# OpenGene/fastplong

Measured on AMD Instinct MI355X. Metric: Gbases/s processed (trim+cut+filter), higher is better.
Workload: dtype u8; 1 GPU; c3_full_pipeline: BASELINE.json configs[2] -- 1000000 synthetic reads per GPU, lognormal lengths (median 8000, sigma 0.5, N50 ~10 kb), Q~N(18,8), -s/-e fixed, --cut_front --cut_tail -W 5, -x, -y; inputs resident in HBM; reads_per_gpu=1000000, bases_per_gpu=9061022094, max_read_len=99450, parallelism=shard1 (independent read shards, one RCCL all-reduce of the counters)

## Files before the change

### fastplong_amd/csrc/dev_prims.h

```cpp
#ifndef FPL_DEV_PRIMS_H
#define FPL_DEV_PRIMS_H

#include <stdint.h>

#ifdef FPL_EMU
#include "hip_emu.h"
#else
#include <hip/hip_runtime.h>
#endif

#ifdef FPL_EMU
#define FPL_NOINLINE
#else
#define FPL_NOINLINE __attribute__((noinline))
#endif

namespace fpl {

constexpr int WAVE = 64;

typedef unsigned long long u64;
typedef uint32_t u32;
typedef uint8_t u8;

// ... 199 lines not shown
    u32 r = 0;
    for (int i = 0; i < 32; i++) {
        const int idx = (((a >> i) & 1) << 2) | (((b >> i) & 1) << 1) | ((c >> i) & 1);
        r |= (u32)((TT >> idx) & 1) << i;
    }
    return r;
#else
    return __builtin_amdgcn_bitop3_b32(a, b, c, TT);
#endif
}
__device__ __forceinline__ void csa(u32& h, u32& l, u32 a, u32 b, u32 c) {
    const u32 hh = bitop3<0xE8>(a, b, c);
    l = bitop3<0x96>(a, b, c);
    h = hh;
}

__device__ __forceinline__ u32 udot4(u32 a, u32 b, u32 c) {
#ifdef FPL_EMU
    u32 r = c;
    for (int i = 0; i < 4; i++) r += ((a >> (8 * i)) & 0xFF) * ((b >> (8 * i)) & 0xFF);
    return r;
#else
    return __builtin_amdgcn_udot4(a, b, c, false);
#endif
}
__device__ __forceinline__ void dot_settle(u32& a, u32& b) {
#ifndef FPL_EMU
    asm volatile("s_nop 3" : "+v"(a), "+v"(b));
#else
    (void)a;
    (void)b;
#endif
}
__device__ __forceinline__ u32 sum_bytes(u32 a, u32 c) {
#ifdef FPL_EMU
    return c + (a & 0xFF) + ((a >> 8) & 0xFF) + ((a >> 16) & 0xFF) + (a >> 24);
#else
    return __builtin_amdgcn_sad_u8(a, 0u, c);
#endif
}
__device__ __forceinline__ u32 perm_lo(u32 tbl, u32 sel) {
#ifdef FPL_EMU
    u32 r = 0;
    for (int i = 0; i < 4; i++) {
        const u32 k = (sel >> (8 * i)) & 0xFF;
        r |= ((k < 4 ? (tbl >> (8 * k)) : 0) & 0xFF) << (8 * i);
    }
    return r;
#else
    return __builtin_amdgcn_perm(0u, tbl, sel);
#endif
}
__device__ __forceinline__ u32 perm_b32(u32 hi, u32 lo, u32 sel) {
#ifdef FPL_EMU
    const u64 v = ((u64)hi << 32) | lo;
    u32 r = 0;
    for (int i = 0; i < 4; i++) {
        const u32 k = (sel >> (8 * i)) & 0xFF;
        r |= (u32)((k < 8 ? (v >> (8 * k)) : 0) & 0xFF) << (8 * i);
    }
    return r;
#else
    return __builtin_amdgcn_perm(hi, lo, sel);
#endif
}
__device__ __forceinline__ u32 uniform_u32(u32 v) {
// ... 76 lines not shown
```

### fastplong_amd/csrc/dev_types.h

```cpp
#ifndef FPL_DEV_TYPES_H
#define FPL_DEV_TYPES_H

#include <math.h>
#include <stdint.h>
#include <string.h>

#include "../../include/fastplong_amd.h"

namespace fpl {

constexpr int PEQ_WORDS = 4;

struct DevAdapter {
    int32_t len;
    int32_t plen;
    uint8_t seq[256];
    uint32_t seqw[256];
    uint32_t peq16_start[256];
    uint32_t peq16_end[256];
    uint64_t peq_full[256][PEQ_WORDS];
    uint32_t term[64];
    int32_t acgt_only;
    uint32_t onehot[8];
    uint64_t peq4_full[4];
    uint32_t peq4_s16[4];
    uint32_t peq4_e16[4];
    uint32_t peq4_e32[4];
    uint32_t peq4_s32r[4];
};

struct DevConfig {
    int32_t trim_front, trim_tail;
    int32_t cut_front, cut_tail;
    int32_t cut_front_w, cut_front_thr;
    int32_t cut_tail_w, cut_tail_thr;
    int32_t polyx, polyx_min_len;
    int32_t adapter_enabled, ext;
    int32_t has_start, has_end, n_fasta;
    int32_t trim_mode;
    int32_t qual_filter, qualified_qual, unqual_pct, n_base_limit, n_pct_limit, avg_qual_req;
    int32_t length_filter, required_length, max_length;
    int32_t complexity, complexity_pct;
    int32_t brk, brk_w, brk_thr, msk, msk_w, msk_thr, defer;
    int32_t dbg;
    int32_t ham_fast;
    int32_t scan_short;
    int32_t thr[FPL_MAX_ADAPTER_LEN + 1];
};

struct ReadState {
    uint32_t s, e;
    uint32_t dropped;
    uint32_t pad;
};

inline void build_adapter(DevAdapter* a, const char* seq, int len) {
    memset(a, 0, sizeof(*a));
    a->len = len;
    a->plen = len < FPL_PATTERN_LEN ? len : FPL_PATTERN_LEN;
    for (int i = 0; i < len; i++) {
        uint8_t c = (uint8_t)seq[i];
        a->seq[i] = c;
        a->seqw[i] = 0x01010101u * c;
        a->peq_full[c][i >> 6] |= 1ull << (i & 63);
    }
    a->acgt_only = len <= 64;
    for (int i = 0; i < 64; i++) a->term[i] = (4u * 4u * 64u) << 8;
    for (int i = 0; i < len && i < 64; i++) {
        const uint8_t c = (uint8_t)seq[i];
        if (c != 'A' && c != 'C' && c != 'G' && c != 'T') a->acgt_only = 0;
        const uint32_t code = (c >> 1) & 3u;
        a->term[i] = ((4u * (code * 64u + (uint32_t)(i >> 5))) << 8) | (uint32_t)(i & 31);
    }
    for (int i = 0; i < len && i < 64; i++) {
        const uint8_t c = (uint8_t)seq[i];
        const uint32_t nib = c == 'A' ? 1u : (c == 'C' ? 2u : (c == 'G' ? 4u : (c == 'T' ? 8u : 0u)));
        a->onehot[i >> 3] |= nib << (4 * (i & 7));
    }
    for (int j = 0; j < a->plen; j++) {
        a->peq16_start[(uint8_t)seq[len - a->plen + j]] |= 1u << j;
        a->peq16_end[(uint8_t)seq[j]] |= 1u << j;
    }
    {
        static const uint8_t letters[4] = {'A', 'C', 'T', 'G'};
        for (int c = 0; c < 4; c++) {
            a->peq4_full[c] = a->peq_full[letters[c]][0];
            a->peq4_s16[c] = a->peq16_start[letters[c]];
            a->peq4_e16[c] = a->peq16_end[letters[c]];
            a->peq4_e32[c] = 0;
            a->peq4_s32r[c] = 0;
            const int m = len < 32 ? len : 32;
            for (int i = 0; i < m; i++) {
                if ((uint8_t)seq[i] == letters[c]) a->peq4_e32[c] |= 1u << i;
                if ((uint8_t)seq[len - 1 - i] == letters[c]) a->peq4_s32r[c] |= 1u << i;
            }
        }
    }
}

inline int trim_mode_of(const int* lens, const int* acgt_only, int n_adapters) {
    bool short_ok = n_adapters == 2, mid_ok = true;
    for (int i = 0; i < n_adapters; i++) {
        const int l = lens[i];
        if (l == 0 && i < 2) continue;
        if (l < 16 || l > 32 || !acgt_only[i]) short_ok = false;
// ... 47 lines not shown
```

### fastplong_amd/csrc/kernels.h

```cpp
#ifndef FPL_KERNELS_H
#define FPL_KERNELS_H

#include "adapter_pick.h"
#include "dev_prims.h"
#include "dev_types.h"

namespace fpl {

#if defined(FPL_PROF) && !defined(FPL_EMU)
__device__ unsigned long long g_fpl_prof[64];
#define PROF_INIT()                                     \
    unsigned long long prof_a[12] = {0, 0, 0, 0, 0, 0, 0, 0, 0, 0, 0, 0}; \
    unsigned long long prof_t = __builtin_amdgcn_s_memtime()
#define PROF(i)                                                     \
    {                                                               \
        const unsigned long long t_ = __builtin_amdgcn_s_memtime(); \
        prof_a[i] += t_ - prof_t;                                   \
        prof_t = t_;                                                \
    }
#define PROF_FLUSH(base)                                                                      \
    if (lane_id() == 0)                                                                       \
        for (int i_ = 0; i_ < 12; i_++) atomicAdd(&g_fpl_prof[(base) + i_], prof_a[i_])
#else
#define PROF_INIT()
// ... 1468 lines not shown
        cC += (c == 'C' || c == 'N');
        cG += (c == 'G' || c == 'N');
        const int cmp = pos + 1, allowed = min(5, cmp / 8);
        const bool need = (cmp - cA > allowed) && (cmp - cT > allowed) && (cmp - cC > allowed) && (cmp - cG > allowed);
        if (need && (pos >= 8 || pos + 1 >= compareReq - 1)) {
            P = pos;
            break;
        }
        pos++;
        if (++it > LANE_SCAN_CAP) slow = true;
    }
    if (!active || slow || P + 1 < compareReq) return rlen;
    int poly = 0, maxc = cA;
    if (cT > maxc) { maxc = cT; poly = 1; }
    if (cC > maxc) { maxc = cC; poly = 2; }
    if (cG > maxc) { maxc = cG; poly = 3; }
    const u32 polyBase = poly == 0 ? 'A' : (poly == 1 ? 'T' : (poly == 2 ? 'C' : 'G'));
    int i = rlen - P - 1;
    if (i < 0) i = 0;
    it = 0;
    while (i < rlen && r[i] != polyBase) {
        i++;
        if (++it > LANE_SCAN_CAP) {
            slow = true;
            return rlen;
        }
    }
    const int p2 = i < rlen ? rlen - i - 1 : -1;
    poly_out = poly;
    trimmed_out = p2 + 1;
    return rlen - p2 - 1;
}

__device__ __forceinline__ u32 onehot4(u32 w) {
    const u32 code = (w >> 1) & 0x03030303u;
    const u32 t = perm_lo(0x47544341u, code) ^ w;
    const u32 ok = (~(((t & 0x7F7F7F7Fu) + 0x7F7F7F7Fu) | t) >> 7) & 0x01010101u;
    const u32 nib = perm_lo(0x04080201u, code) & (ok * 15u);
    const u32 h = (nib | (nib >> 4)) & 0x00FF00FFu;
    return (h | (h >> 8)) & 0xFFFFu;
}
template <bool START, int NW = 4>
__device__ __forceinline__ void ham_scan_lanes(const u8* __restrict__ r1, int rlen, bool active, const u32 (&ad1h)[NW], int alen,
                                               int thr, const u8* __restrict__ seq_end, int& hit, int& cand) {
    hit = -1;
    cand = -1;
    int p_lo = 0, np = 0;
    if (START) {
        const int searchEnd = min(rlen, FPL_END_WINDOW);
        if (active && alen <= rlen && searchEnd > alen) np = searchEnd - alen + 1;
    } else {
        const int ss = max(0, rlen - FPL_END_WINDOW);
        if (active && ss + alen <= rlen) {
            p_lo = ss;
            np = rlen - alen - ss;
        }
    }
    const int npmax = (int)wave_max_u32((u32)max(np, 0));
    if (npmax == 0) return;
    const u8* base = r1 + p_lo;
    const int navail = np > 0 ? rlen - p_lo : 0;
    auto nibbles = [&](int k) -> u32 {
        const int left = navail - 4 * k;
        if (left <= 0) return 0u;
        u32 w = load4_guard(base + 4 * k, seq_end);
        if (left < 4) w &= (1u << (8 * left)) - 1u;
        return onehot4(w);
    };
    u32 touch = 0;
    if (navail > 64)
        touch = (u32)*(base + min(navail - 1, 112)) + (u32)*(base + min(navail - 1, 207));
    u32 W[NW];
#pragma unroll
    for (int k = 0; k < NW; k++) W[k] = nibbles(2 * k) | (nibbles(2 * k + 1) << 16);
    int bestmm = 0x7fffffff;
    u32 nxt = nibbles(2 * NW);
    for (int i0 = 0; i0 < npmax; i0 += 4) {
        const u32 cur = nxt;
        nxt = nibbles(i0 / 4 + 2 * NW + 1);
#pragma unroll
        for (int u = 0; u < 4; u++) {
            const int i = i0 + u;
            u32 matches = popc32(W[0] & ad1h[0]);
#pragma unroll
            for (int k = 1; k < NW; k++) matches = popc_acc(W[k] & ad1h[k], matches);
            const int mm = alen - (int)matches;
            const bool in = i < np;
            const int p = p_lo + i;
            if (START) {
                hit = (in && mm <= thr) ? p : hit;
                const bool better = in && mm < bestmm;
                cand = better ? p : cand;
                bestmm = better ? mm : bestmm;
            } else {
                hit = (in && hit < 0 && mm <= thr) ? p : hit;
                const bool better = in && mm <= bestmm;
                cand = better ? p : cand;
                bestmm = better ? mm : bestmm;
            }
#pragma unroll
            for (int k = 0; k + 1 < NW; k++) W[k] = alignbit(W[k + 1], W[k], 4);
            W[NW - 1] = (W[NW - 1] >> 4) | (((cur >> (4 * u)) & 15u) << 28);
        }
    }
    if (hit >= 0) cand = -1;
#if !defined(FPL_EMU)
    asm volatile("" ::"v"(touch));
#else
    (void)touch;
#endif
}

__device__ __forceinline__ bool lev_lanes32(const u8* __restrict__ text, int m, int shift, int thr, bool need,
                                            const uint64_t (*__restrict__ peqf)[1], const u8* __restrict__ seq_end) {
    u32 w[8] = {0, 0, 0, 0, 0, 0, 0, 0};
    if (need) {
        const u32x4 a = load16_guard(text, seq_end), b = load16_guard(text + 16, seq_end);
        w[0] = a.x; w[1] = a.y; w[2] = a.z; w[3] = a.w;
        w[4] = b.x; w[5] = b.y; w[6] = b.z; w[7] = b.w;
    }
    const int mm = need ? m : 0;
    const u32 mask = mm >= 32 ? ~0u : ((1u << mm) - 1u);
    const u32 topsh = mm > 0 ? (u32)(mm - 1) : 0u;
    const int mmax = (int)wave_max_u32((u32)mm);
    u32 Pv = ~0u, Mv = 0;
    int score = mm;
#pragma unroll
    for (int t = 0; t < 32; t++) {
        if (t < mmax) {
            const u32 c = (w[t >> 2] >> (8 * (t & 3))) & 0xFFu;
            const u32 Eq = (u32)(peqf[c][0] >> shift) & mask;
            const u32 Xv = Eq | Mv;
            const u32 Xh = (((Eq & Pv) + Pv) ^ Pv) | Eq;
            u32 Ph = Mv | ~(Xh | Pv);
            u32 Mh = Pv & Xh;
            const int sc = score + (int)((Ph >> topsh) & 1u) - (int)((Mh >> topsh) & 1u);
            Ph = (Ph << 1) | 1u;
            Mh <<= 1;
            const bool act = t < mm;
            score = act ? sc : score;
            const u32 nPv = Mh | ~(Xv | Ph), nMv = Ph & Xv;
            Pv = act ? nPv : Pv;
            Mv = act ? nMv : Mv;
        }
// ... 159 lines not shown
        if (ok && ed <= thrP) {
            if (START) {
                if (ed < mined) {
                    mined = ed;
                    pos = p;
                }
            } else if (pos < 0 || ed <= mined) {
                pos = p;
                mined = ed;
            } else {
                stop = true;
            }
        }
        if (stop) {
            cur = 0;
            nz = 0;
        }
    }
    return pos;
}

__device__ __forceinline__ int lane_get(int v, int j) { return readlane_i32(v, j); }
__device__ __forceinline__ void lane_set(int& v, int j, int x) { v = lane_id() == j ? x : v; }

#ifndef FPL_TRIM_WAVES_PER_SIMD_BATCHED
#define FPL_TRIM_WAVES_PER_SIMD_BATCHED 5
#endif
template <int WAVES, int NW = 4, bool CHAIN = false>
__global__ void __launch_bounds__(WAVES * 64, FPL_TRIM_WAVES_PER_SIMD_BATCHED)
k_trim_ends_batched(const u8* __restrict__ seq, const u8* __restrict__ qual, const uint64_t* __restrict__ off, u32 n_reads,
                    uint64_t n_bytes, const DevConfig* __restrict__ cfg, const DevAdapter* __restrict__ ads,
                    ReadState* __restrict__ state, long long* __restrict__ counters, u32 C, u32* __restrict__ group_ctr) {
    __shared__ TrimBlockAcc acc;
    __shared__ TrimLds<WAVES> lds;
    __shared__ int thr_lds[72];
    __shared__ u32 cand_lds[WAVES][PART_WORDS][64];
    PROF_INIT();
    const int lane = lane_id();
    u32(*const cand)[64] = cand_lds[wave_in_block()];
    for (u32 i = threadIdx.x; i < FPL_FR_LEN; i += blockDim.x) acc.fr[i] = 0;
    for (u32 i = threadIdx.x; i < 2 * 2 * FPL_KEY_STRIDE; i += blockDim.x) acc.key[i] = 0;
    for (u32 i = threadIdx.x; i < 256; i += blockDim.x) {
        lds.peq16[0][i] = (uint16_t)ads[0].peq16_start[i];
        lds.peq16[1][i] = (uint16_t)ads[1].peq16_end[i];
        lds.peqf[0][i][0] = ads[0].peq_full[i][0];
        lds.peqf[1][i][0] = ads[1].peq_full[i][0];
    }
    for (u32 i = threadIdx.x; i < 72; i += blockDim.x) thr_lds[i] = i <= 64 ? cfg->thr[i] : 0;
    __syncthreads();
    const u8* seq_end = seq + n_bytes;
    const u8* qual_end = qual + n_bytes;
    u32* const win_s = lds.win[wave_in_block()][0];
    u32* const win_e = lds.win[wave_in_block()][1];
    u32* const win_hq = lds.win[wave_in_block()][2];
    u32* const win_tq = lds.win[wave_in_block()][3];
    u32* const win4_s = lds.win4[wave_in_block()][0];
    u32* const win4_e = lds.win4[wave_in_block()][1];
    const bool do_ad = cfg->adapter_enabled != 0;
    const bool do_start = do_ad && cfg->has_start, do_end = do_ad && cfg->has_end;
    const int ext = cfg->ext;
    const int alen0 = ads[0].len, alen1 = ads[1].len;
    constexpr int plen = FPL_PATTERN_LEN;
    const int thrA0 = cfg->thr[alen0], thrA1 = cfg->thr[alen1], thrP = cfg->thr[plen];
    u32 ad1h0[NW], ad1h1[NW];
#pragma unroll
    for (int k = 0; k < NW; k++) {
        ad1h0[k] = uniform_u32(ads[0].onehot[k]);
        ad1h1[k] = uniform_u32(ads[1].onehot[k]);
    }

    const u32 n_groups = (n_reads + 63) / 64;
    for (;;) {
        u32 grp = 0;
        if (lane == 0) grp = atomicAdd(group_ctr, 1u);
        grp = readlane_u32(grp, 0);
        if (grp >= n_groups) break;
        const u32 g0 = grp * 64;
        const int gn = (int)min(64u, n_reads - g0);
        FPL_TRIM_STAT(0, 1);
        uint64_t v_o0 = 0;
        int v_l = 0;
        if (lane < gn) {
            v_o0 = off[g0 + lane];
            v_l = (int)(off[g0 + lane + 1] - v_o0);
        }
        int v_s = 0, v_e = 0, v_alive = 0, v_trim = 0;
        int v_mpos = -1;
        int v_cand = -1;

        PROF(0)
        bool v_slow = false;
        {
            bool alive = false, slow = false;
            const bool wide = (cfg->cut_front && cfg->cut_front_w > LANE_SCAN_WMAX) || (cfg->cut_tail && cfg->cut_tail_w > LANE_SCAN_WMAX);
            if (!wide) {
                trim_and_cut_lanes(seq + v_o0, qual + v_o0, v_l, lane < gn, cfg, v_s, v_e, alive, slow);
                if (cfg->polyx) {
                    int poly, tl;
                    const int nl = trim_polyx_lanes(seq + v_o0 + v_s, v_e - v_s, alive && !slow, cfg->polyx_min_len, poly, tl, slow);
                    if (!slow) {
                        v_e = v_s + nl;
                        if (poly >= 0) {
// ... 9 lines not shown
            v_slow = slow;
        }
        PROF(1)
        for (u64 todo = wave_ballot(v_slow); todo;) {
            const int j = __ffsll(todo) - 1;
            todo &= todo - 1;
            FPL_TRIM_STAT(1, 1);
            const uint64_t o0 = readlane_u64(v_o0, j);
            const int l = lane_get(v_l, j);
            const u8* sq = seq + o0;
            const u8* ql = qual + o0;
            const int tail0 = max(0, l - TRIM_WIN);
            stage_ends<true>(win_s, win_e, win_hq, win_tq, win4_s, win4_e, sq, ql, l, tail0, seq_end, qual_end);
            const EndsView vs = {sq, (const u8*)win_s, (const u8*)win_e, tail0};
            const EndsView vq = {ql, (const u8*)win_hq, (const u8*)win_tq, tail0};
            int s, e;
            const bool alive = trim_and_cut_wave(vs, vq, l, cfg, s, e);
            if (alive && cfg->polyx) {
                int poly, tl;
                const int nl = trim_polyx_wave(vs, s, e - s, cfg->polyx_min_len, poly, tl);
                e = s + nl;
                if (poly >= 0 && lane == 0) {
                    atomicAdd(&acc.fr[FPL_FR_POLYX_READS + poly], (u64)1);
                    atomicAdd(&acc.fr[FPL_FR_POLYX_BASES + poly], (u64)tl);
                }
            }
            lane_set(v_s, j, s);
            lane_set(v_e, j, e);
            lane_set(v_alive, j, alive ? 1 : 0);
        }
        PROF(2)
        if (do_start) {
            const bool act = v_alive && (v_e - v_s) >= FPL_PATTERN_LEN;
            ham_scan_lanes<true, NW>(seq + v_o0 + v_s, v_e - v_s, act, ad1h0, alen0, thrA0, seq_end, v_mpos, v_cand);
        }
        PROF(3)
        if (do_start) {
            const bool need = v_cand >= 0;
            FPL_TRIM_STAT(2, __popcll(wave_ballot(need)));
            if (wave_ballot(need)) {
                const bool ok = lev_lanes_nw<NW>(seq + v_o0 + v_s + v_cand, alen0, 0, thrA0, need, lds.peqf[0], seq_end);
                v_mpos = ok ? v_cand : v_mpos;
            }
        }
        PROF(4)
        int v_ppos = -1;
        if (do_start) {
            const int rl = v_e - v_s;
            const bool wants = v_alive && v_mpos < 0 && rl >= FPL_PATTERN_LEN;
            bool may = false;
            if (wave_ballot(wants)) {
                const int n = min(rl, FPL_END_WINDOW);
                const u32 nzc = partial16_candidates(seq + v_o0 + v_s, n, thrP, wants, lds.peq16[0], seq_end, cand);
                if (wave_ballot(nzc != 0))
                    v_ppos = partial16_resolve_lanes<true>(seq + v_o0 + v_s, n, min(rl - plen, FPL_END_WINDOW - plen), thrP, nzc,
                                                           lds.peq16[0], seq_end, cand, may);
            }
            u64 todo = wave_ballot(may);
            FPL_TRIM_STAT(3, __popcll(wave_ballot(wants)));
            FPL_TRIM_STAT(4, __popcll(todo));
            while (todo) {
                const int j = __ffsll(todo) - 1;
                todo &= todo - 1;
                const uint64_t o0 = readlane_u64(v_o0, j);
                const int s = lane_get(v_s, j), e = lane_get(v_e, j), rlen = e - s;
                const u8* sq = seq + o0;
                stage_window(win_s, sq + s, min(rlen, FPL_END_WINDOW), seq_end, nullptr);
// ... 18 lines not shown
            }
        }
        PROF(5)
        if (do_start) {
            const int rlen = v_e - v_s;
            const int cmplen = min(v_ppos + plen, alen0);
            const bool need = v_ppos >= 0;
            bool pok = false;
            if (wave_ballot(need))
                pok = lev_lanes_nw<NW>(seq + v_o0 + v_s + v_ppos + plen - cmplen, cmplen, alen0 - cmplen, thr_lds[need ? cmplen : 0], need,
                                  lds.peqf[0], seq_end);
            int kl = 0, got = 0;
            if (v_mpos >= 0) {
                const int mp = min(v_mpos + ext, rlen - alen0);
                kl = alen0;
                v_s += min(rlen - 1, mp + alen0);
                got = mp + alen0;
            } else if (pok) {
                const int pos = min(v_ppos + ext, rlen - alen0);
                kl = cmplen;
                const int n = min(rlen - 1, pos + plen);
                if (n < 0) v_s = v_e;
                else v_s += n;
                got = pos + plen;
            }
            v_trim += got;
            if (kl > 0) atomicAdd(&acc.key[(0 * 2 + 0) * FPL_KEY_STRIDE + kl], 1u);
        }
        PROF(6)
        v_mpos = -1;
        v_cand = -1;
        if (do_end) {
            const bool act = v_alive && (v_e - v_s) >= FPL_PATTERN_LEN;
            ham_scan_lanes<false, NW>(seq + v_o0 + v_s, v_e - v_s, act, ad1h1, alen1, thrA1, seq_end, v_mpos, v_cand);
        }
        PROF(7)
        if (do_end) {
            const bool need = v_cand >= 0;
            FPL_TRIM_STAT(5, __popcll(wave_ballot(need)));
            if (wave_ballot(need)) {
                const bool ok = lev_lanes_nw<NW>(seq + v_o0 + v_s + v_cand, alen1, 0, thrA1, need, lds.peqf[1], seq_end);
                v_mpos = ok ? v_cand : v_mpos;
            }
        }
        PROF(8)
        v_ppos = -1;
        if (do_end) {
            const int rl = v_e - v_s, wlf = min(rl, FPL_END_WINDOW);
            const bool wants = v_alive && v_mpos < 0 && rl >= FPL_PATTERN_LEN;
            bool may = false;
            if (wave_ballot(wants)) {
                const u32 nzc = partial16_candidates(seq + v_o0 + v_e - wlf, wlf, thrP, wants, lds.peq16[1], seq_end, cand);
                if (wave_ballot(nzc != 0)) {
                    const int pos = partial16_resolve_lanes<false>(seq + v_o0 + v_e - 16, wlf, min(rl - plen, FPL_END_WINDOW - plen), thrP,
                                                                   nzc, lds.peq16[1], seq_end, cand, may);
                    v_ppos = pos > 0 ? pos : -1;
                }
            }
            u64 todo = wave_ballot(may);
            FPL_TRIM_STAT(6, __popcll(wave_ballot(wants)));
            FPL_TRIM_STAT(7, __popcll(todo));
            while (todo) {
                const int j = __ffsll(todo) - 1;
                todo &= todo - 1;
                const uint64_t o0 = readlane_u64(v_o0, j);
                const int s = lane_get(v_s, j), e = lane_get(v_e, j), rlen = e - s;
                const u8* sq = seq + o0;
// ... 46 lines not shown
                v_e = v_s + mp;
                got = rlen - mp;
            } else if (pok) {
                const int pos = min(v_ppos + ext, rlen - plen);
                kl = cmplen;
                v_e = v_s + (rlen - plen - pos);
                got = pos + plen;
            }
            v_trim += got;
            if (kl > 0) atomicAdd(&acc.key[(1 * 2 + 1) * FPL_KEY_STRIDE + kl], 1u);
        }
        if (do_ad && !CHAIN) {
            const u64 nt = wave_ballot(v_trim > 0);
            const u32 tb = wave_sum_u32(v_trim > 0 ? (u32)v_trim : 0u);
            if (nt && lane == 0) {
                atomicAdd(&acc.fr[FPL_FR_ADAPTER_READS], (u64)__popcll(nt));
                atomicAdd(&acc.fr[FPL_FR_ADAPTER_BASES], (u64)tb);
            }
        }
        if (lane < gn) {
            ReadState st;
            st.s = v_alive ? (u32)v_s : 0;
            st.e = v_alive ? (u32)v_e : 0;
            st.dropped = v_alive ? 0 : 1;
            st.pad = CHAIN ? (u32)v_trim : 0u;
            state[g0 + lane] = st;
        }
        PROF(10)
    }
    PROF_FLUSH(32);
    __syncthreads();
    long long* fr = counters + FPL_OFF_FR(C);
    long long* keyh = counters + FPL_OFF_KEYHIST(C);
    for (u32 i = threadIdx.x; i < FPL_FR_LEN; i += blockDim.x)
        if (acc.fr[i]) atomicAdd((u64*)&fr[i], acc.fr[i]);
    for (u32 i = threadIdx.x; i < 2 * 2 * FPL_KEY_STRIDE; i += blockDim.x)
        if (acc.key[i]) atomicAdd((u64*)&keyh[i], (u64)acc.key[i]);
}

constexpr int FS_T = 512;
constexpr int FS_SMAX = 96;
constexpr int FS_PT = FS_T + FS_SMAX;
constexpr int FS_SLAB = 8 * FS_T + 8 * FS_PT;
constexpr int FS_STRIDE = FS_T + FS_PT;
__device__ __forceinline__ u32 fs_pre_cell(u32 i) { return (i / FS_T) * FS_STRIDE + (i % FS_T); }
__device__ __forceinline__ u32 fs_post_cell(u32 j) { return (j / FS_PT) * FS_STRIDE + FS_T + (j % FS_PT); }
constexpr u32 CS_MAX_ITEMS_PER_SLICE = 16383;
#ifndef FPL_ABL
#define FPL_ABL 0
#endif
constexpr int CS_GROUP = 4;
constexpr u32 PLAN_TO_POST = 1u;

__device__ __forceinline__ u32 kmer_codes(u32 d) { return (d & 0x02020202u) | ((d >> 2) & 0x01010101u); }
__device__ __forceinline__ u32 kmer_pack(u32 v) {
    const u32 x = lshl_or<10>(v, v);
    return lshl_or<20>(x, x);
}
__device__ __forceinline__ u32 kmer_pack_dot(u32 v) { return udot4(v, 0x01041040u, 0u); }
__device__ __forceinline__ u32 kmer_stream(u32 v0, u32 v1, u32 pack_h0) {
    u32 p0 = kmer_pack_dot(v0), p1 = kmer_pack_dot(v1);
    dot_settle(p0, p1);
    const u32 W01 = lshl_or<8>(p0, p1);
    return lshl_or<16>(wave_prev_u32(W01, pack_h0), W01);
}
__device__ __forceinline__ u32 invalid_nibble(u32 mapped, u32 d) {
    const u32 x = (mapped ^ d) & ~((mapped >> 4) & 0x01010101u);
    const u32 nz = (((x & 0x7F7F7F7Fu) + 0x7F7F7F7Fu) | x) & 0x80808080u;
    const u32 y = lshl_or<7>(nz, nz);
// ... 499 lines not shown
                    const u32 mm = (acc[j >> 2] >> (8 * (j & 3))) & 0xFF;
                    if (j0 + j < npos0 && mm < bmm0) {
                        bmm0 = mm;
                        bp0 = (u32)(j0 + j);
                    }
                }
            }
            if (npos1 > t0) {
                hamming16(rb + a + j0, seq_end, sv, ad1->seqw, ad1->len, acc);
#pragma unroll
                for (int j = 0; j < 16; j++) {
                    const u32 mm = (acc[j >> 2] >> (8 * (j & 3))) & 0xFF;
                    if (j0 + j < npos1 && mm < bmm1) {
                        bmm1 = mm;
                        bp1 = (u32)(j0 + j);
                    }
                }
            }
        }
    }
    if (SUMS) {
        sums.lowq = wave_sum_u32(lowq);
        sums.nn = wave_sum_u32(nn);
        sums.totq = wave_sum_u32(totq);
        sums.diff = wave_sum_u32(diff);
    }
    if (HAM) {
        key0 = wave_min_u64(((u64)bmm0 << 32) | bp0);
        key1 = wave_min_u64(((u64)bmm1 << 32) | bp1);
    }
}


__device__ __forceinline__ void code_planes(const u32 s[8], u32& L, u32& H, u32& N) {
    L = 0;
    H = 0;
    N = 0;
#pragma unroll
    for (int pr = 0; pr < 4; pr++) {
        u32 lb = 0, hb = 0, nb = 0;
#pragma unroll
        for (int hh = 0; hh < 2; hh++) {
            const u32 w = s[2 * pr + hh];
            const u32 wt = hh ? 0x80402010u : 0x08040201u;
            lb = udot4(w & 0x02020202u, wt, lb);
            hb = udot4(w & 0x04040404u, wt, hb);
            nb = udot4(w & 0x08080808u, wt, nb);
        }
        L |= pr ? lb << (8 * pr - 1) : lb >> 1;
        H |= pr ? hb << (8 * pr - 2) : hb >> 2;
        N |= pr ? nb << (8 * pr - 3) : nb >> 3;
    }
}
__device__ __forceinline__ u32 not_acgtn(const u32 s[8]) {
    u32 bad = 0;
#pragma unroll
    for (int d = 0; d < 8; d++) bad |= perm_b32(0x4E000000u, 0x47544341u, (s[d] >> 1) & 0x07070707u) ^ s[d];
    return bad;
}
template <bool MASKED, bool QS = true>
__device__ __forceinline__ void sums32_acgtn(const u32 s0, const u32 q[8], int nvalid, u32 L, u32 H, u32 N, u32 prev_dword,
                                             u32 qqrep, u32& lowq, u32& nn, u32& totq, u32& diff) {
#pragma unroll
    for (int d = 0; QS && d < 8; d++) {
        u32 bm = ~0u, fm = 0x80808080u;
        if (MASKED) {
            const int c = nvalid - 4 * d;
            bm = c >= 4 ? ~0u : (c <= 0 ? 0u : ((1u << (8 * c)) - 1u));
            fm &= bm;
        }
        const u32 t = (q[d] | 0x80808080u) - qqrep;
        lowq = popc_acc(~t & fm, lowq);
        totq = sum_bytes(q[d] & bm, totq);
    }
    const u32 vm = (!MASKED || nvalid >= 32) ? ~0u : ((1u << nvalid) - 1u);
    nn = popc_acc(N & vm, nn);
    const u32 dm = ((L ^ (L << 1)) | (H ^ (H << 1)) | (N ^ (N << 1))) & ~1u & vm;
    const u32 d0 = ((s0 & 0xFFu) != (prev_dword >> 24)) ? 1u : 0u;
    diff = popc_acc(dm, diff) + d0;
}
__device__ __forceinline__ void build_planes(const u32 s[8], u32& PA, u32& PC, u32& PT, u32& PG) {
    u32 L = 0, H = 0, X = 0;
#pragma unroll
    for (int pr = 0; pr < 4; pr++) {
        u32 lb = 0, hb = 0, xb = 0;
#pragma unroll
        for (int hh = 0; hh < 2; hh++) {
            const u32 w = s[2 * pr + hh];
            const u32 wt = hh ? 0x80402010u : 0x08040201u;
            const u32 w1 = w >> 1;
            lb = udot4(w1 & 0x01010101u, wt, lb);
            hb = udot4((w >> 2) & 0x01010101u, wt, hb);
            const u32 e = perm_lo(0x47544341u, w1 & 0x03030303u);
            const u32 t = e ^ w;
            const u32 nz = ((((t & 0x7F7F7F7Fu) + 0x7F7F7F7Fu) | t) >> 7) & 0x01010101u;
            xb = udot4(nz, wt, xb);
        }
        L |= lb << (8 * pr);
        H |= hb << (8 * pr);
        X |= xb << (8 * pr);
    }
    const u32 V = ~X;
    PA = bitop3<0x10>(V, H, L);
    PC = bitop3<0x20>(V, H, L);
    PT = bitop3<0x40>(V, H, L);
    PG = bitop3<0x80>(V, H, L);
}

template <int NB>
__device__ __forceinline__ void match_counts(const u32* __restrict__ plane_lane, const DevAdapter* __restrict__ ad, u32 (&B)[NB]) {
    const int alen = ad->len;
#ifndef FPL_EMU
    const u32 planes_m0 = uniform_u32((u32)(size_t)plane_lane - 4u * (u32)lane_id());
#endif
#pragma unroll
    for (int b = 0; b < NB; b++) B[b] = 0;
    auto group8 = [&](int i0) -> u32 {
        u32 m[8], tw[8];
#pragma unroll
        for (int k = 0; k < 8; k++) tw[k] = ad->term[i0 + k];
#ifdef FPL_EMU
#pragma unroll
        for (int k = 0; k < 8; k++) {
            const u32* p = plane_lane + (tw[k] >> 10);
            m[k] = alignbit(p[1], p[0], tw[k] & 31u);
        }
#else
        u32 lo[8], hi[8], m0_keep;
        asm volatile(
            "s_mov_b32 %16, m0\n"
            "s_lshr_b32 m0, %17, 8\n s_add_u32 m0, m0, %25\n s_nop 0\n ds_read_addtid_b32 %0 offset:0\n ds_read_addtid_b32 %8 offset:4\n"
            "s_lshr_b32 m0, %18, 8\n s_add_u32 m0, m0, %25\n s_nop 0\n ds_read_addtid_b32 %1 offset:0\n ds_read_addtid_b32 %9 offset:4\n"
            "s_lshr_b32 m0, %19, 8\n s_add_u32 m0, m0, %25\n s_nop 0\n ds_read_addtid_b32 %2 offset:0\n ds_read_addtid_b32 %10 offset:4\n"
            "s_lshr_b32 m0, %20, 8\n s_add_u32 m0, m0, %25\n s_nop 0\n ds_read_addtid_b32 %3 offset:0\n ds_read_addtid_b32 %11 offset:4\n"
            "s_lshr_b32 m0, %21, 8\n s_add_u32 m0, m0, %25\n s_nop 0\n ds_read_addtid_b32 %4 offset:0\n ds_read_addtid_b32 %12 offset:4\n"
            "s_lshr_b32 m0, %22, 8\n s_add_u32 m0, m0, %25\n s_nop 0\n ds_read_addtid_b32 %5 offset:0\n ds_read_addtid_b32 %13 offset:4\n"
            "s_lshr_b32 m0, %23, 8\n s_add_u32 m0, m0, %25\n s_nop 0\n ds_read_addtid_b32 %6 offset:0\n ds_read_addtid_b32 %14 offset:4\n"
            "s_lshr_b32 m0, %24, 8\n s_add_u32 m0, m0, %25\n s_nop 0\n ds_read_addtid_b32 %7 offset:0\n ds_read_addtid_b32 %15 offset:4\n"
            "s_waitcnt lgkmcnt(0)\n s_mov_b32 m0, %16"
            : "=&v"(lo[0]), "=&v"(lo[1]), "=&v"(lo[2]), "=&v"(lo[3]), "=&v"(lo[4]), "=&v"(lo[5]), "=&v"(lo[6]), "=&v"(lo[7]),
              "=&v"(hi[0]), "=&v"(hi[1]), "=&v"(hi[2]), "=&v"(hi[3]), "=&v"(hi[4]), "=&v"(hi[5]), "=&v"(hi[6]), "=&v"(hi[7]),
              "=&s"(m0_keep)
            : "s"(tw[0]), "s"(tw[1]), "s"(tw[2]), "s"(tw[3]), "s"(tw[4]), "s"(tw[5]), "s"(tw[6]), "s"(tw[7]), "s"(planes_m0)
            : "scc", "memory");
        (void)m0_keep;
#pragma unroll
        for (int k = 0; k < 8; k++) m[k] = alignbit(hi[k], lo[k], tw[k]);
#endif
        u32 t1, t2, t3, t4, f1, f2, e;
        csa(t1, B[0], B[0], m[0], m[1]);
        csa(t2, B[0], B[0], m[2], m[3]);
        csa(f1, B[1], B[1], t1, t2);
        csa(t3, B[0], B[0], m[4], m[5]);
        csa(t4, B[0], B[0], m[6], m[7]);
        csa(f2, B[1], B[1], t3, t4);
        csa(e, B[2], B[2], f1, f2);
        return e;
    };
    auto ripple = [&](u32 c, int lvl) {
#pragma unroll
        for (int b = 3; b < NB; b++) {
            if (b < lvl) continue;
            const u32 t = B[b] & c;
            B[b] ^= c;
            c = t;
        }
    };
    int i0 = 0;
    for (; i0 + 8 < alen; i0 += 16) {
        const u32 ea = group8(i0);
        const u32 eb = group8(i0 + 8);
        u32 c16;
        csa(c16, B[3], B[3], ea, eb);
        ripple(c16, 4);
    }
    for (; i0 < alen; i0 += 8) ripple(group8(i0), 3);
}

template <int NB>
__device__ __forceinline__ void sliced_max(const u32 (&B)[NB], u32 cand, int& val, int& first) {
    val = 0;
#pragma unroll
    for (int b = NB - 1; b >= 0; b--) {
        const u32 t = cand & B[b];
        const bool nz = t != 0;
        cand = nz ? t : cand;
#ifndef FPL_EMU
        {
            u64 c = wave_ballot(nz);
            asm("s_nop 1\n\tv_addc_co_u32_e64 %0, %1, %0, %0, %1" : "+v"(val), "+s"(c));
        }
#else
        val = val + val + (nz ? 1 : 0);
#endif
    }
    first = __ffs(cand) - 1;
}

template <bool MASKED, bool QS = true>
__device__ __forceinline__ void sums32(const u32 s[8], const u32 q[8], int nvalid, u32 prev_dword, u32 qqrep, u32& lowq,
                                       u32& nn, u32& totq, u32& diff) {
    u32 pd = prev_dword;
#pragma unroll
    for (int d = 0; d < 8; d++) {
        u32 bm = ~0u, fm = 0x80808080u;
        if (MASKED) {
            const int c = nvalid - 4 * d;
            bm = c >= 4 ? ~0u : (c <= 0 ? 0u : ((1u << (8 * c)) - 1u));
            fm &= bm;
        }
        if (QS) {
            const u32 t = (q[d] | 0x80808080u) - qqrep;
            lowq = popc_acc(~t & fm, lowq);
            totq = sum_bytes(q[d] & bm, totq);
        }
        const u32 x = s[d] ^ 0x4E4E4E4Eu;
        const u32 zx = ((x & 0x7F7F7F7Fu) + 0x7F7F7F7Fu) | x;
        nn = popc_acc(~zx & fm, nn);
        const u32 y = s[d] ^ alignbyte(s[d], pd, 3);
        const u32 zy = ((y & 0x7F7F7F7Fu) + 0x7F7F7F7Fu) | y;
        diff = popc_acc(zy & fm, diff);
        pd = s[d];
    }
}
struct HistLane {
    u32* p;
    u32 addr;
};
__device__ __forceinline__ HistLane hist_lane(u32* __restrict__ h) {
// ... 176 lines not shown
        prev_tile_last = readlane_u32(s[7], ACTIVE - 1);
        if (j0 == 0) prevd = s[0] << 24;
        bool acgt = false;
        u32 cL = 0, cH = 0, cN = 0;
        if (!LEAN && (SUMS || HAM)) {
            acgt = !wave_ballot(not_acgtn(s) != 0);
            if (acgt) code_planes(s, cL, cH, cN);
        }
        if (!LEAN) {
            if (nstat > 0) {
                if (!FPL_DBG(dbg, 1) && !head) hist32<false>(hl, q, SC_CHUNK);
                if (SUMS && !FPL_DBG(dbg, 2)) {
                    if (packed) {
                        u32 t_nn = head ? 0u : nn, t_diff = head ? 0u : diff;
                        if (acgt) sums32_acgtn<false, false>(s[0], q, SC_CHUNK, cL, cH, cN, prevd, qqrep, lowq, t_nn, totq, t_diff);
                        else sums32<false, false>(s, q, SC_CHUNK, prevd, qqrep, lowq, t_nn, totq, t_diff);
                        h_nn = head ? t_nn : 0u;
                        h_diff = head ? t_diff : 0u;
                        nn = head ? nn : t_nn;
                        diff = head ? diff : t_diff;
                    } else if (acgt) sums32_acgtn<false, false>(s[0], q, SC_CHUNK, cL, cH, cN, prevd, qqrep, lowq, nn, totq, diff);
                    else sums32<false, false>(s, q, SC_CHUNK, prevd, qqrep, lowq, nn, totq, diff);
                }
                if (FPL_DBG(dbg, 4)) totq += s[0] + s[3] + s[4] + s[7] + q[0] + q[3] + q[4] + q[7];
            }
        } else if (nstat > 0) {
            hist32<true>(hl, q, nstat);
            if (SUMS) sums32<true>(s, q, nstat, prevd, qqrep, lowq, nn, totq, diff);
        }
        if (HAM) {
            if ((npos0 > t0 || npos1 > t0 || packed) && !FPL_DBG(dbg, 16)) {
                u32 PA, PC, PT, PG;
                if (acgt) {
                    PA = ~(cH | cL);
                    PC = ~cH & cL;
                    PT = cH & ~cL;
                    PG = cH & cL & ~cN;
                } else {
                    build_planes(s, PA, PC, PT, PG);
                }
                wave_sync();
                w->planes[0][lane] = PA;
                w->planes[1][lane] = PC;
                w->planes[2][lane] = PT;
                w->planes[3][lane] = PG;
                wave_sync();
                const u32* plane_lane = &w->planes[0][lane < ACTIVE ? lane : 0];
                u32 B[NB];
                if ((npos0 > t0 || packed) && !FPL_DBG(dbg, 8)) {
                    match_counts(plane_lane, ad0, B);
                    u32 vm = act_mask;
                    if (npos0 - t0 < ACTIVE * SC_CHUNK) {
                        const int nv = npos0 - j0;
                        vm = (lane >= ACTIVE || nv <= 0) ? 0u : (nv >= 32 ? 0xFFFFFFFFu : ((1u << nv) - 1u));
                    }
                    if (head) vm = act_mask;
                    if (vm) {
                        int val, first;
                        sliced_max(B, vm, val, first);
                        if (packed && head) {
                            h_bm0 = val;
                            h_bp0 = j0 + first;
                        } else if (val > bm0) {
                            bm0 = val;
                            bp0 = j0 + first;
                        }
                    }
                }
                if ((npos1 > t0 || packed) && !FPL_DBG(dbg, 8)) {
                    match_counts(plane_lane, ad1, B);
// ... 1718 lines not shown
```

Before: 798.8 Gbases/s.

## Replace per-lane nibble Hamming scan with bit-sliced plane ring-buffer matcher

```diff
diff --git a/fastplong_amd/csrc/dev_prims.h b/fastplong_amd/csrc/dev_prims.h
--- a/fastplong_amd/csrc/dev_prims.h
+++ b/fastplong_amd/csrc/dev_prims.h
@@ -255,6 +255,15 @@
     (void)b;
 #endif
 }
+__device__ __forceinline__ void dot_settle(u32& a, u32& b, u32& c) {
+#ifndef FPL_EMU
+    asm volatile("s_nop 3" : "+v"(a), "+v"(b), "+v"(c));
+#else
+    (void)a;
+    (void)b;
+    (void)c;
+#endif
+}
 __device__ __forceinline__ u32 sum_bytes(u32 a, u32 c) {
 #ifdef FPL_EMU
     return c + (a & 0xFF) + ((a >> 8) & 0xFF) + ((a >> 16) & 0xFF) + (a >> 24);
diff --git a/fastplong_amd/csrc/dev_types.h b/fastplong_amd/csrc/dev_types.h
--- a/fastplong_amd/csrc/dev_types.h
+++ b/fastplong_amd/csrc/dev_types.h
@@ -27,6 +27,7 @@
     uint32_t peq4_e16[4];
     uint32_t peq4_e32[4];
     uint32_t peq4_s32r[4];
+    uint32_t term_own[64];
 };
 
 struct DevConfig {
@@ -65,12 +66,13 @@
         a->peq_full[c][i >> 6] |= 1ull << (i & 63);
     }
     a->acgt_only = len <= 64;
-    for (int i = 0; i < 64; i++) a->term[i] = (4u * 4u * 64u) << 8;
+    for (int i = 0; i < 64; i++) a->term[i] = a->term_own[i] = (4u * 4u * 64u) << 8;
     for (int i = 0; i < len && i < 64; i++) {
         const uint8_t c = (uint8_t)seq[i];
         if (c != 'A' && c != 'C' && c != 'G' && c != 'T') a->acgt_only = 0;
         const uint32_t code = (c >> 1) & 3u;
         a->term[i] = ((4u * (code * 64u + (uint32_t)(i >> 5))) << 8) | (uint32_t)(i & 31);
+        a->term_own[i] = ((4u * code * 64u) << 8) | (uint32_t)(i & 31);
     }
     for (int i = 0; i < len && i < 64; i++) {
         const uint8_t c = (uint8_t)seq[i];
diff --git a/fastplong_amd/csrc/kernels.h b/fastplong_amd/csrc/kernels.h
--- a/fastplong_amd/csrc/kernels.h
+++ b/fastplong_amd/csrc/kernels.h
@@ -1524,84 +1524,15 @@
     return rlen - p2 - 1;
 }
 
-__device__ __forceinline__ u32 onehot4(u32 w) {
-    const u32 code = (w >> 1) & 0x03030303u;
-    const u32 t = perm_lo(0x47544341u, code) ^ w;
-    const u32 ok = (~(((t & 0x7F7F7F7Fu) + 0x7F7F7F7Fu) | t) >> 7) & 0x01010101u;
-    const u32 nib = perm_lo(0x04080201u, code) & (ok * 15u);
-    const u32 h = (nib | (nib >> 4)) & 0x00FF00FFu;
-    return (h | (h >> 8)) & 0xFFFFu;
-}
+template <int NW>
+struct HamScanPark {
+    static constexpr int RING = NW <= 4 ? 2 : 3;
+    u32 w[RING + 1][5][64];
+};
 template <bool START, int NW = 4>
-__device__ __forceinline__ void ham_scan_lanes(const u8* __restrict__ r1, int rlen, bool active, const u32 (&ad1h)[NW], int alen,
-                                               int thr, const u8* __restrict__ seq_end, int& hit, int& cand) {
-    hit = -1;
-    cand = -1;
-    int p_lo = 0, np = 0;
-    if (START) {
-        const int searchEnd = min(rlen, FPL_END_WINDOW);
-        if (active && alen <= rlen && searchEnd > alen) np = searchEnd - alen + 1;
-    } else {
-        const int ss = max(0, rlen - FPL_END_WINDOW);
-        if (active && ss + alen <= rlen) {
-            p_lo = ss;
-            np = rlen - alen - ss;
-        }
-    }
-    const int npmax = (int)wave_max_u32((u32)max(np, 0));
-    if (npmax == 0) return;
-    const u8* base = r1 + p_lo;
-    const int navail = np > 0 ? rlen - p_lo : 0;
-    auto nibbles = [&](int k) -> u32 {
-        const int left = navail - 4 * k;
-        if (left <= 0) return 0u;
-        u32 w = load4_guard(base + 4 * k, seq_end);
-        if (left < 4) w &= (1u << (8 * left)) - 1u;
-        return onehot4(w);
-    };
-    u32 touch = 0;
-    if (navail > 64)
-        touch = (u32)*(base + min(navail - 1, 112)) + (u32)*(base + min(navail - 1, 207));
-    u32 W[NW];
-#pragma unroll
-    for (int k = 0; k < NW; k++) W[k] = nibbles(2 * k) | (nibbles(2 * k + 1) << 16);
-    int bestmm = 0x7fffffff;
-    u32 nxt = nibbles(2 * NW);
-    for (int i0 = 0; i0 < npmax; i0 += 4) {
-        const u32 cur = nxt;
-        nxt = nibbles(i0 / 4 + 2 * NW + 1);
-#pragma unroll
-        for (int u = 0; u < 4; u++) {
-            const int i = i0 + u;
-            u32 matches = popc32(W[0] & ad1h[0]);
-#pragma unroll
-            for (int k = 1; k < NW; k++) matches = popc_acc(W[k] & ad1h[k], matches);
-            const int mm = alen - (int)matches;
-            const bool in = i < np;
-            const int p = p_lo + i;
-            if (START) {
-                hit = (in && mm <= thr) ? p : hit;
-                const bool better = in && mm < bestmm;
-                cand = better ? p : cand;
-                bestmm = better ? mm : bestmm;
-            } else {
-                hit = (in && hit < 0 && mm <= thr) ? p : hit;
-                const bool better = in && mm <= bestmm;
-                cand = better ? p : cand;
-                bestmm = better ? mm : bestmm;
-            }
-#pragma unroll
-            for (int k = 0; k + 1 < NW; k++) W[k] = alignbit(W[k + 1], W[k], 4);
-            W[NW - 1] = (W[NW - 1] >> 4) | (((cur >> (4 * u)) & 15u) << 28);
-        }
-    }
-    if (hit >= 0) cand = -1;
-#if !defined(FPL_EMU)
-    asm volatile("" ::"v"(touch));
-#else
-    (void)touch;
-#endif
-}
+__device__ __forceinline__ void ham_scan_lanes(const u8* __restrict__ r1, int rlen, bool active, const DevAdapter* __restrict__ ad,
+                                               int alen, int thr, const u8* __restrict__ seq_end, HamScanPark<NW>& park, int& hit,
+                                               int& cand);
 
 __device__ __forceinline__ bool lev_lanes32(const u8* __restrict__ text, int m, int shift, int thr, bool need,
                                             const uint64_t (*__restrict__ peqf)[1], const u8* __restrict__ seq_end) {
@@ -1827,12 +1758,25 @@
                     uint64_t n_bytes, const DevConfig* __restrict__ cfg, const DevAdapter* __restrict__ ads,
                     ReadState* __restrict__ state, long long* __restrict__ counters, u32 C, u32* __restrict__ group_ctr) {
     __shared__ TrimBlockAcc acc;
-    __shared__ TrimLds<WAVES> lds;
+    struct AdapterLds {
+        uint16_t peq16[2][256];
+        uint64_t peqf[2][256][1];
+    };
+    __shared__ AdapterLds lds;
     __shared__ int thr_lds[72];
-    __shared__ u32 cand_lds[WAVES][PART_WORDS][64];
+    union WaveLds {
+        HamScanPark<NW> park;
+        struct {
+            u32 cand[PART_WORDS][64];
+            u32 win[4][TRIM_WIN / 4 + 8];
+            u32 win4[2][TRIM_WIN / 8 + 8];
+        } rd;
+    };
+    __shared__ WaveLds wave_lds[WAVES];
     PROF_INIT();
     const int lane = lane_id();
-    u32(*const cand)[64] = cand_lds[wave_in_block()];
+    u32(*const cand)[64] = wave_lds[wave_in_block()].rd.cand;
+    HamScanPark<NW>& park = wave_lds[wave_in_block()].park;
     for (u32 i = threadIdx.x; i < FPL_FR_LEN; i += blockDim.x) acc.fr[i] = 0;
     for (u32 i = threadIdx.x; i < 2 * 2 * FPL_KEY_STRIDE; i += blockDim.x) acc.key[i] = 0;
     for (u32 i = threadIdx.x; i < 256; i += blockDim.x) {
@@ -1845,24 +1789,18 @@
     __syncthreads();
     const u8* seq_end = seq + n_bytes;
     const u8* qual_end = qual + n_bytes;
-    u32* const win_s = lds.win[wave_in_block()][0];
-    u32* const win_e = lds.win[wave_in_block()][1];
-    u32* const win_hq = lds.win[wave_in_block()][2];
-    u32* const win_tq = lds.win[wave_in_block()][3];
-    u32* const win4_s = lds.win4[wave_in_block()][0];
-    u32* const win4_e = lds.win4[wave_in_block()][1];
+    u32* const win_s = wave_lds[wave_in_block()].rd.win[0];
+    u32* const win_e = wave_lds[wave_in_block()].rd.win[1];
+    u32* const win_hq = wave_lds[wave_in_block()].rd.win[2];
+    u32* const win_tq = wave_lds[wave_in_block()].rd.win[3];
+    u32* const win4_s = wave_lds[wave_in_block()].rd.win4[0];
+    u32* const win4_e = wave_lds[wave_in_block()].rd.win4[1];
     const bool do_ad = cfg->adapter_enabled != 0;
     const bool do_start = do_ad && cfg->has_start, do_end = do_ad && cfg->has_end;
     const int ext = cfg->ext;
     const int alen0 = ads[0].len, alen1 = ads[1].len;
     constexpr int plen = FPL_PATTERN_LEN;
     const int thrA0 = cfg->thr[alen0], thrA1 = cfg->thr[alen1], thrP = cfg->thr[plen];
-    u32 ad1h0[NW], ad1h1[NW];
-#pragma unroll
-    for (int k = 0; k < NW; k++) {
-        ad1h0[k] = uniform_u32(ads[0].onehot[k]);
-        ad1h1[k] = uniform_u32(ads[1].onehot[k]);
-    }
 
     const u32 n_groups = (n_reads + 63) / 64;
     for (;;) {
@@ -1938,7 +1876,7 @@
         PROF(2)
         if (do_start) {
             const bool act = v_alive && (v_e - v_s) >= FPL_PATTERN_LEN;
-            ham_scan_lanes<true, NW>(seq + v_o0 + v_s, v_e - v_s, act, ad1h0, alen0, thrA0, seq_end, v_mpos, v_cand);
+            ham_scan_lanes<true, NW>(seq + v_o0 + v_s, v_e - v_s, act, &ads[0], alen0, thrA0, seq_end, park, v_mpos, v_cand);
         }
         PROF(3)
         if (do_start) {
@@ -2023,7 +1961,7 @@
         v_cand = -1;
         if (do_end) {
             const bool act = v_alive && (v_e - v_s) >= FPL_PATTERN_LEN;
-            ham_scan_lanes<false, NW>(seq + v_o0 + v_s, v_e - v_s, act, ad1h1, alen1, thrA1, seq_end, v_mpos, v_cand);
+            ham_scan_lanes<false, NW>(seq + v_o0 + v_s, v_e - v_s, act, &ads[1], alen1, thrA1, seq_end, park, v_mpos, v_cand);
         }
         PROF(7)
         if (do_end) {
@@ -2136,9 +2074,11 @@
     __syncthreads();
     long long* fr = counters + FPL_OFF_FR(C);
     long long* keyh = counters + FPL_OFF_KEYHIST(C);
-    for (u32 i = threadIdx.x; i < FPL_FR_LEN; i += blockDim.x)
+    u32 tid = threadIdx.x;
+    opaque_u32(tid);
+    for (u32 i = tid; i < FPL_FR_LEN; i += blockDim.x)
         if (acc.fr[i]) atomicAdd((u64*)&fr[i], acc.fr[i]);
-    for (u32 i = threadIdx.x; i < 2 * 2 * FPL_KEY_STRIDE; i += blockDim.x)
+    for (u32 i = tid; i < 2 * 2 * FPL_KEY_STRIDE; i += blockDim.x)
         if (acc.key[i]) atomicAdd((u64*)&keyh[i], (u64)acc.key[i]);
 }
 
@@ -2704,6 +2644,7 @@
 }
 
 
+template <bool SETTLE = false>
 __device__ __forceinline__ void code_planes(const u32 s[8], u32& L, u32& H, u32& N) {
     L = 0;
     H = 0;
@@ -2719,10 +2660,17 @@
             hb = udot4(w & 0x04040404u, wt, hb);
             nb = udot4(w & 0x08080808u, wt, nb);
         }
+        if (SETTLE) dot_settle(lb, hb, nb);
         L |= pr ? lb << (8 * pr - 1) : lb >> 1;
         H |= pr ? hb << (8 * pr - 2) : hb >> 2;
         N |= pr ? nb << (8 * pr - 3) : nb >> 3;
     }
+}
+__device__ __forceinline__ void letter_planes(u32 cL, u32 cH, u32 cN, u32& PA, u32& PC, u32& PT, u32& PG) {
+    PA = ~(cH | cL);
+    PC = ~cH & cL;
+    PT = cH & ~cL;
+    PG = cH & cL & ~cN;
 }
 __device__ __forceinline__ u32 not_acgtn(const u32 s[8]) {
     u32 bad = 0;
@@ -2751,6 +2699,7 @@
     const u32 d0 = ((s0 & 0xFFu) != (prev_dword >> 24)) ? 1u : 0u;
     diff = popc_acc(dm, diff) + d0;
 }
+template <bool SETTLE = false>
 __device__ __forceinline__ void build_planes(const u32 s[8], u32& PA, u32& PC, u32& PT, u32& PG) {
     u32 L = 0, H = 0, X = 0;
 #pragma unroll
@@ -2768,6 +2717,7 @@
             const u32 nz = ((((t & 0x7F7F7F7Fu) + 0x7F7F7F7Fu) | t) >> 7) & 0x01010101u;
             xb = udot4(nz, wt, xb);
         }
+        if (SETTLE) dot_settle(lb, hb, xb);
         L |= lb << (8 * pr);
         H |= hb << (8 * pr);
         X |= xb << (8 * pr);
@@ -2779,41 +2729,43 @@
     PG = bitop3<0x80>(V, H, L);
 }
 
-template <int NB>
-__device__ __forceinline__ void match_counts(const u32* __restrict__ plane_lane, const DevAdapter* __restrict__ ad, u32 (&B)[NB]) {
+template <int NB, int HI_OFF = 4, bool OWN = false>
+__device__ __forceinline__ void match_counts(const u32* __restrict__ plane_lane, const DevAdapter* __restrict__ ad, u32 (&B)[NB],
+                                             int adj32 = 0) {
     const int alen = ad->len;
 #ifndef FPL_EMU
-    const u32 planes_m0 = uniform_u32((u32)(size_t)plane_lane - 4u * (u32)lane_id());
+    const u32 planes_m0_lo = uniform_u32((u32)(size_t)plane_lane - 4u * (u32)lane_id());
 #endif
 #pragma unroll
     for (int b = 0; b < NB; b++) B[b] = 0;
     auto group8 = [&](int i0) -> u32 {
         u32 m[8], tw[8];
 #pragma unroll
-        for (int k = 0; k < 8; k++) tw[k] = ad->term[i0 + k];
+        for (int k = 0; k < 8; k++) tw[k] = OWN ? ad->term_own[i0 + k] : ad->term[i0 + k];
 #ifdef FPL_EMU
 #pragma unroll
         for (int k = 0; k < 8; k++) {
-            const u32* p = plane_lane + (tw[k] >> 10);
-            m[k] = alignbit(p[1], p[0], tw[k] & 31u);
+            const u32* p = plane_lane + (tw[k] >> 10) + (i0 >= 32 ? adj32 / 4 : 0);
+            m[k] = alignbit(p[HI_OFF / 4], p[0], tw[k] & 31u);
         }
 #else
         u32 lo[8], hi[8], m0_keep;
+        const u32 planes_m0 = planes_m0_lo + (u32)(i0 >= 32 ? adj32 : 0);
         asm volatile(
             "s_mov_b32 %16, m0\n"
-            "s_lshr_b32 m0, %17, 8\n s_add_u32 m0, m0, %25\n s_nop 0\n ds_read_addtid_b32 %0 offset:0\n ds_read_addtid_b32 %8 offset:4\n"
-            "s_lshr_b32 m0, %18, 8\n s_add_u32 m0, m0, %25\n s_nop 0\n ds_read_addtid_b32 %1 offset:0\n ds_read_addtid_b32 %9 offset:4\n"
-            "s_lshr_b32 m0, %19, 8\n s_add_u32 m0, m0, %25\n s_nop 0\n ds_read_addtid_b32 %2 offset:0\n ds_read_addtid_b32 %10 offset:4\n"
-            "s_lshr_b32 m0, %20, 8\n s_add_u32 m0, m0, %25\n s_nop 0\n ds_read_addtid_b32 %3 offset:0\n ds_read_addtid_b32 %11 offset:4\n"
-            "s_lshr_b32 m0, %21, 8\n s_add_u32 m0, m0, %25\n s_nop 0\n ds_read_addtid_b32 %4 offset:0\n ds_read_addtid_b32 %12 offset:4\n"
-            "s_lshr_b32 m0, %22, 8\n s_add_u32 m0, m0, %25\n s_nop 0\n ds_read_addtid_b32 %5 offset:0\n ds_read_addtid_b32 %13 offset:4\n"
-            "s_lshr_b32 m0, %23, 8\n s_add_u32 m0, m0, %25\n s_nop 0\n ds_read_addtid_b32 %6 offset:0\n ds_read_addtid_b32 %14 offset:4\n"
-            "s_lshr_b32 m0, %24, 8\n s_add_u32 m0, m0, %25\n s_nop 0\n ds_read_addtid_b32 %7 offset:0\n ds_read_addtid_b32 %15 offset:4\n"
+            "s_lshr_b32 m0, %17, 8\n s_add_u32 m0, m0, %25\n s_nop 0\n ds_read_addtid_b32 %0 offset:0\n ds_read_addtid_b32 %8 offset:%26\n"
+            "s_lshr_b32 m0, %18, 8\n s_add_u32 m0, m0, %25\n s_nop 0\n ds_read_addtid_b32 %1 offset:0\n ds_read_addtid_b32 %9 offset:%26\n"
+            "s_lshr_b32 m0, %19, 8\n s_add_u32 m0, m0, %25\n s_nop 0\n ds_read_addtid_b32 %2 offset:0\n ds_read_addtid_b32 %10 offset:%26\n"
+            "s_lshr_b32 m0, %20, 8\n s_add_u32 m0, m0, %25\n s_nop 0\n ds_read_addtid_b32 %3 offset:0\n ds_read_addtid_b32 %11 offset:%26\n"
+            "s_lshr_b32 m0, %21, 8\n s_add_u32 m0, m0, %25\n s_nop 0\n ds_read_addtid_b32 %4 offset:0\n ds_read_addtid_b32 %12 offset:%26\n"
+            "s_lshr_b32 m0, %22, 8\n s_add_u32 m0, m0, %25\n s_nop 0\n ds_read_addtid_b32 %5 offset:0\n ds_read_addtid_b32 %13 offset:%26\n"
+            "s_lshr_b32 m0, %23, 8\n s_add_u32 m0, m0, %25\n s_nop 0\n ds_read_addtid_b32 %6 offset:0\n ds_read_addtid_b32 %14 offset:%26\n"
+            "s_lshr_b32 m0, %24, 8\n s_add_u32 m0, m0, %25\n s_nop 0\n ds_read_addtid_b32 %7 offset:0\n ds_read_addtid_b32 %15 offset:%26\n"
             "s_waitcnt lgkmcnt(0)\n s_mov_b32 m0, %16"
             : "=&v"(lo[0]), "=&v"(lo[1]), "=&v"(lo[2]), "=&v"(lo[3]), "=&v"(lo[4]), "=&v"(lo[5]), "=&v"(lo[6]), "=&v"(lo[7]),
               "=&v"(hi[0]), "=&v"(hi[1]), "=&v"(hi[2]), "=&v"(hi[3]), "=&v"(hi[4]), "=&v"(hi[5]), "=&v"(hi[6]), "=&v"(hi[7]),
               "=&s"(m0_keep)
-            : "s"(tw[0]), "s"(tw[1]), "s"(tw[2]), "s"(tw[3]), "s"(tw[4]), "s"(tw[5]), "s"(tw[6]), "s"(tw[7]), "s"(planes_m0)
+            : "s"(tw[0]), "s"(tw[1]), "s"(tw[2]), "s"(tw[3]), "s"(tw[4]), "s"(tw[5]), "s"(tw[6]), "s"(tw[7]), "s"(planes_m0), "n"(HI_OFF)
             : "scc", "memory");
         (void)m0_keep;
 #pragma unroll
@@ -2849,7 +2801,7 @@
     for (; i0 < alen; i0 += 8) ripple(group8(i0), 3);
 }
 
-template <int NB>
+template <int NB, bool LAST = false>
 __device__ __forceinline__ void sliced_max(const u32 (&B)[NB], u32 cand, int& val, int& first) {
     val = 0;
 #pragma unroll
@@ -2867,6 +2819,127 @@
 #endif
     }
     first = __ffs(cand) - 1;
+    if (LAST) first = 31 - (int)__clz((int)cand);
+}
+template <int NB>
+__device__ __forceinline__ u32 sliced_ge(const u32 (&B)[NB], int t) {
+    const u32 k = (1u << NB) - (u32)t;
+    u32 c = 0;
+#pragma unroll
+    for (int b = 0; b < NB; b++) c = bitop3<0xE8>(B[b], c, ((k >> b) & 1u) ? ~0u : 0u);
+    return c;
+}
+
+template <bool START, int NW>
+__device__ __forceinline__ void ham_scan_lanes(const u8* __restrict__ r1, int rlen, bool active, const DevAdapter* __restrict__ ad,
+                                               int alen, int thr, const u8* __restrict__ seq_end, HamScanPark<NW>& park, int& hit,
+                                               int& cand) {
+    constexpr int NB = NW <= 4 ? 6 : 7;
+    constexpr int RING = HamScanPark<NW>::RING;
+    constexpr int SLOT = (int)sizeof(park.w[0]);
+    constexpr int NWORDS = (FPL_END_WINDOW + 31) / 32;
+    hit = -1;
+    cand = -1;
+    int p_lo = 0, np = 0;
+    int navail = 0;
+    if (START) {
+        const int searchEnd = min(rlen, FPL_END_WINDOW);
+        if (active && alen <= rlen && searchEnd > alen) {
+            np = searchEnd - alen + 1;
+            navail = searchEnd;
+        }
+    } else {
+        const int ss = max(0, rlen - FPL_END_WINDOW);
+        if (active && ss + alen <= rlen) {
+            p_lo = ss;
+            np = rlen - alen - ss;
+            navail = np > 0 ? rlen - ss : 0;
+        }
+    }
+    const int npmax = (int)wave_max_u32((u32)max(np, 0));
+    if (npmax == 0) return;
+    const int nwo = (npmax + 31) >> 5;
+    const int nww = min(NWORDS, ((int)wave_max_u32((u32)navail) + 31) >> 5);
+    const u8* base = r1 + p_lo;
+    auto fetch = [&](int w, u32 (&s)[8]) {
+        if (32 * w < navail) {
+            const u32x4 a = load16_guard(base + 32 * w, seq_end), b = load16_guard(base + 32 * w + 16, seq_end);
+            s[0] = a.x; s[1] = a.y; s[2] = a.z; s[3] = a.w;
+            s[4] = b.x; s[5] = b.y; s[6] = b.z; s[7] = b.w;
+        } else {
+#pragma unroll
+            for (int d = 0; d < 8; d++) s[d] = 0x41414141u;
+        }
+    };
+    const int lane = lane_id();
+    u32* const pl = &park.w[0][0][lane];
+    auto put = [&](int w, const u32 (&s)[8]) {
+        u32 PA = 0, PC = 0, PT = 0, PG = 0;
+        if (w < nww) {
+            if (!wave_ballot(not_acgtn(s) != 0)) {
+                u32 cL, cH, cN;
+                code_planes<true>(s, cL, cH, cN);
+                letter_planes(cL, cH, cN, PA, PC, PT, PG);
+            } else {
+                build_planes<true>(s, PA, PC, PT, PG);
+            }
+            const int n = navail - 32 * w;
+            const u32 in = n >= 32 ? ~0u : (n <= 0 ? 0u : ((1u << n) - 1u));
+            PA &= in;
+            PC &= in;
+            PT &= in;
+            PG &= in;
+        }
+        u32* const q = pl + (w % RING) * (SLOT / 4);
+        q[0 * 64] = PA;
+        q[1 * 64] = PC;
+        q[2 * 64] = PT;
+        q[3 * 64] = PG;
+        if (w % RING == 0) {
+            u32* const q2 = pl + RING * (SLOT / 4);
+            q2[0 * 64] = PA;
+            q2[1 * 64] = PC;
+            q2[2 * 64] = PT;
+            q2[3 * 64] = PG;
+        }
+    };
+#pragma unroll
+    for (int k = 0; k <= RING; k++) pl[k * (SLOT / 4) + 4 * 64] = 0;
+    u32 s[8];
+#pragma unroll
+    for (int w = 0; w < RING - 1; w++) {
+        fetch(w, s);
+        put(w, s);
+    }
+    fetch(RING - 1, s);
+    const int need = alen - thr;
+    int best = -1;
+    for (int j = 0; j < nwo; j++) {
+        put(j + RING - 1, s);
+        if (j + 1 < nwo) fetch(j + RING, s);
+        u32 B[NB];
+        const int s0 = j % RING, s1 = (j + 1) % RING;
+        match_counts<NB, SLOT, true>(pl + s0 * (SLOT / 4), ad, B, (s1 - s0) * SLOT);
+        const int nv = np - 32 * j;
+        const u32 vm = nv >= 32 ? ~0u : (nv <= 0 ? 0u : ((1u << nv) - 1u));
+        const u32 hm = need > 0 ? sliced_ge(B, need) & vm : vm;
+        const int p0 = p_lo + 32 * j;
+        int val, pos;
+        if (START) {
+            hit = hm ? p0 + 31 - (int)__clz((int)hm) : hit;
+            sliced_max<NB, false>(B, vm, val, pos);
+            const bool better = vm != 0 && val > best;
+            cand = better ? p0 + pos : cand;
+            best = better ? val : best;
+        } else {
+            hit = (hm && hit < 0) ? p0 + (int)__ffs((int)hm) - 1 : hit;
+            sliced_max<NB, true>(B, vm, val, pos);
+            const bool better = vm != 0 && val >= best;
+            cand = better ? p0 + pos : cand;
+            best = better ? val : best;
+        }
+    }
+    if (hit >= 0) cand = -1;
 }
 
 template <bool MASKED, bool QS = true>
@@ -3109,10 +3182,7 @@
             if ((npos0 > t0 || npos1 > t0 || packed) && !FPL_DBG(dbg, 16)) {
                 u32 PA, PC, PT, PG;
                 if (acgt) {
-                    PA = ~(cH | cL);
-                    PC = ~cH & cL;
-                    PT = cH & ~cL;
-                    PG = cH & cL & ~cN;
+                    letter_planes(cL, cH, cN, PA, PC, PT, PG);
                 } else {
                     build_planes(s, PA, PC, PT, PG);
                 }
```

Result: faster. 814.7 Gbases/s, median of 6 (+2.0%).
